# mitrefireline/simfire

Measured on AMD Instinct MI355X. Metric: cell-updates/sec (grid x envs x steps), higher is better.
Workload: dtype u8 status + u8 sprite masks + f64 burn_amounts

## Files before the change

profiles/run_timeline.py:

```python
import ctypes
import sys

import numpy as np

sys.path.insert(0, ".")
from simfire_amd import workloads
from simfire_amd.engine import FireEngine

NAMES = {15: "step start", 1: "interest+ranks", 2: "list+barrierA", 3: "cursor+next fetch issued", 11: "rows arrived", 4: "nb masks, strips",
         5: "SWAR, stores issued", 6: "prefix+frontier list", 7: "walk: winner", 8: "walk: burn/table arrived, update", 9: "walk: stores, fence",
         10: "end of batch", 0: "barrier B (end of step)", 12: "fold", 13: "lines: eligible bits + barrier", 14: "lines: plane work issued", 16: "first batch known", 17: "its rows requested", 18: "next batch known",
         20: "win start", 21: "win rows arrived", 22: "win frontier known", 23: "win winners+req", 24: "win table arrived", 25: "win updated", 26: "win at barrier",
         27: "win thru barrier", 28: "win folded", 30: "launch start", 31: "fire found", 32: "window loaded", 33: "updates done", 34: "written back",
         35: "steps done", 36: "handed back", 37: "result block", 41: "slot written", 42: "placed", 43: "loads issued", 44: "LDS filled",
         45: "cells stored", 46: "bitmap stored", 47: "hist updated", 48: "row written", 49: "state committed",
         50: "lines applied", 51: "next classified", 52: "lines start"}


def main():
    steps, warm = int(sys.argv[1]), int(sys.argv[2])
    env = int(sys.argv[3]) if len(sys.argv) > 3 else -1
    envs = int(sys.argv[4]) if len(sys.argv) > 4 else 256
    c5 = len(sys.argv) > 5 and sys.argv[5] in ("c5", "c3mit")
    c3mit = len(sys.argv) > 5 and sys.argv[5] == "c3mit"
    c4 = len(sys.argv) > 5 and sys.argv[5] == "c4"
    w = workloads.c5(1024, envs) if c5 and not c3mit else (workloads.c4(2048, envs) if c4 else workloads.c3(1024, envs))
    pts = None
    if c3mit:
        pts = np.zeros((steps + warm, w.n_envs, 64, 3), dtype=np.int32)
    elif c5:
        H, W = w.shape
        pts = np.ascontiguousarray(workloads.agent_walk(w.n_envs, w.agents_per_env, H, W, steps + warm).reshape(
            steps + warm, w.n_envs, w.agents_per_env, 4)[..., 1:])

    def run(eng, a, b):
        if c5:
            eng.step_mitigated(pts[a:b])
        else:
            eng.step(b - a)
    eng = FireEngine(M_f=w.M_f, device=0, **w.engine_kwargs())
    eng.set_layers(*w.layers())
    L = eng._L
    L.sf_debug_timeline.argtypes = [ctypes.c_int32, ctypes.c_int32, ctypes.c_void_p]
    L.sf_debug_wave_log.argtypes = [ctypes.c_int32, ctypes.c_void_p]
    log = np.zeros((16384, 4), dtype=np.uint64)
    if env < 0:
        eng.reset(w.init_xy)
        run(eng, 0, warm)
        L.sf_debug_wave_log(1, None)
        run(eng, warm, warm + steps)
        eng.status()
        L.sf_debug_wave_log(0, log.ctypes.data_as(ctypes.c_void_p))
        env = int(np.argmax(log[:envs, 0]))
        print("slowest env", env, "clocks", int(log[env, 0]), "vectors", int(log[env, 1]))
    eng.reset(w.init_xy)
    run(eng, 0, warm)
    L.sf_debug_timeline(env, -1 if len(sys.argv) > 6 and sys.argv[6] == "launch" else steps - 1, None)
    run(eng, warm, warm + steps)
    eng.status()
    tl = np.zeros((16, 64), dtype=np.uint64)
    L.sf_debug_timeline(0, 0, tl.ctypes.data_as(ctypes.c_void_p))
    t0 = min(int(v & np.uint64(0x00FFFFFFFFFFFFFF)) for v in tl[:, 0] if v)
    for wv in range(16):
        ev = [(int(v >> np.uint64(56)), int(v & np.uint64(0x00FFFFFFFFFFFFFF)) - t0) for v in tl[wv] if v]
        print("wave %2d: " % wv + "  ".join("%s@%d" % (NAMES.get(k, str(k)).split(":")[0].split(",")[0][:14], t) for k, t in ev))


if __name__ == "__main__":
    main()
```

simfire_amd/csrc/sf_common.h:

```cpp
#pragma once
#include <hip/hip_runtime.h>

#include <cstdint>

#include "../../include/simfire_hip.h"
#include "../../include/simfire_hip_lab.h"

namespace {


#ifndef SF_WAVES_PER_SIMD
#define SF_WAVES_PER_SIMD 1
#endif
#ifndef SF_WAVES_PER_GROUP
#define SF_WAVES_PER_GROUP 4
#endif
constexpr int kWaves = SF_WAVES_PER_GROUP;
constexpr int kListCap = 384;
constexpr int kSeamPad = 8;
constexpr int kCounterShards = 256;
constexpr int kCounterRow = 16;
constexpr uint32_t FLAG_LIVE = 1u;
constexpr uint32_t FLAG_CAND = 0x100u;

// ... 22 lines not shown
    int Hs;
    long long seam_env;
    int prune_after_quit;
    int VW;
    long long vb_env;
    long long cells_env;
};

__host__ __device__ inline int bl_vec(const Geo &g, int y, int v)
{
    return ((y >> 2) * g.PV + v) * 128 + ((y >> 1) & 1) * 64;
}
__host__ __device__ inline int bl_cell(const Geo &g, int y, int x)
{
    return bl_vec(g, y, x >> 4) + (y & 1) * 16 + (x & 15);
}
constexpr int kBlStatus = 32;

constexpr uint32_t kLoopStop = 0x80000000u;
constexpr uint32_t kJoinClosed = 0x80000000u;
constexpr int kJoinLog = 4096;
constexpr int kTeamMax = 4;
constexpr uint32_t kTeamUnused = 0xFFFFFFFFu;
__host__ __device__ inline int team_xrow(const Geo &g) { return (64 + g.PV * 16 + 127) / 128 * 128; }

struct StepArgs {
    Geo g;
    uint8_t *status;
    uint8_t *age;
    uint8_t *cells;
    double *burn;
    const double *rt;
    unsigned long long *win_hint;
    const double *rtc;
    EnvState *commit;
    EnvState *tmp;
    uint32_t *flags;
    unsigned long long *counters;
    uint8_t *tflags;
    int ring;
    uint32_t *tile_list;
    uint32_t *n_active;
    uint32_t *settled;
    uint8_t *seam;
    uint8_t *tdirty;
    uint8_t *parents;
// ... 186 lines not shown
```

simfire_amd/csrc/sf_run_kernels.h:

```cpp
#pragma once

#include "sf_common.h"
#include "sf_step_kernels.h"

namespace {

constexpr int kMarkDw = 32;
constexpr int kStripDw = 19;
#ifdef SF_NO_PERM_ELIG
#define ELIG(x) elig01(x)
#else
#define ELIG(x) elig01_perm(x)
#endif
constexpr int kRunCtl = 24;
constexpr int kRunMaxD = 4;

typedef uint32_t __attribute__((aligned(1))) u32_unaligned;
typedef uint32_t u32x4 __attribute__((ext_vector_type(4)));

__host__ __device__ inline size_t win_lds_bytes(int n_waves)
{
    const int WR = n_waves * 4;
    return (size_t)WR * 64 * 8 + 8 * 8 * 4 + 128 * 4 + 64 * 4 + (size_t)(WR + 2) * 18 * 4 + (size_t)WR * 16 + (size_t)2 * WR * 64 * 2 + (size_t)2 * WR * 64 +
           (size_t)WR * 64 + (size_t)WR * 8 + 256 * 4;
}
__host__ __device__ inline size_t run_strip_dwords(int n_waves)
{
    const size_t strips = (size_t)n_waves * (64 * kStripDw + kMarkDw), win = (win_lds_bytes(n_waves) + 15) / 16 * 4;
    return strips > win ? strips : win;
}

__host__ __device__ inline size_t run_lds_bytes(const Geo &g, int n_waves, int vcap, int team = 0, int team_rcap = 0)
{
    const int maps = (team || g.VW == 1) ? 4 : 1;
    const int rows = team && team_rcap ? team_rcap + 2 : g.H;
    size_t b = (size_t)maps * rows * g.VW * 8 + (size_t)vcap * 4 + run_strip_dwords(n_waves) * 4 + kRunCtl * 4;
    if (team) b += (size_t)2 * g.PV * 16 + 64 * 4;
// ... 483 lines not shown
        if (TEAM && (tn > 1 || a.team_rcap) && general) fits = cut_bands(tn > 1 && a.team_recut > 0 && a.team_recut < n_steps ? a.team_recut : n_steps - s_begin);
        if (TEAM && a.todo_out && tm == 0 && tid == 0) a.todo_out[e] = fits ? 0 : n_steps - s_begin;
        if (TEAM && !fits) {
            if (!a.todo_out && tid == 0) *reinterpret_cast<volatile uint32_t *>(a.xerr) = 1u;
            if (s_begin > 0 && tm == 0 && tid == 0) a.commit[e] = st;
            return;
        }
    }
    bool has_up = TEAM && tm > 0, has_dn = TEAM && tm + 1 < tn;
    if (TEAM == 2 && tm == 0 && j_s0 < 0 && tid == 0)
        __hip_atomic_store(a.xj + 2 * g.E + 2 + e, (uint32_t)__builtin_amdgcn_s_getreg((20 << 0) | (0 << 6) | (31 << 11)) & 15u, __ATOMIC_RELAXED, __HIP_MEMORY_SCOPE_AGENT);
    auto team_release = [&]() {
        if (TEAM == 2 && a.join_local == 1) asm volatile("s_waitcnt vmcnt(0)" ::: "memory");
        else __builtin_amdgcn_fence(__ATOMIC_RELEASE, "agent");
    };
    auto team_acquire = [&]() { __builtin_amdgcn_fence(__ATOMIC_ACQUIRE, "agent"); };
    bool one_l2 = false;
    bool gave_up = false;
    auto line_up = [&](const uint32_t tag, const bool report) {
        typedef unsigned long long u64;
        int lane = threadIdx.x & 63;
        asm volatile("" : "+v"(lane));
        const uint32_t xcc = (uint32_t)__builtin_amdgcn_s_getreg((20 << 0) | (0 << 6) | (31 << 11)) & 15u;
        if (lane == 0) __hip_atomic_store(a.xg + ((size_t)e * kTeamMax + tm) * 3 + 2, ((u64)tag << 32) | (u64)xcc, __ATOMIC_RELAXED, __HIP_MEMORY_SCOPE_AGENT);
        u64 x = ((u64)tag << 32) | xcc;
        const unsigned long long t0 = __builtin_amdgcn_s_memrealtime();
        for (;;) {
            if (lane < tn) x = __hip_atomic_load(a.xg + ((size_t)e * kTeamMax + lane) * 3 + 2, __ATOMIC_RELAXED, __HIP_MEMORY_SCOPE_AGENT);
            if (__all((uint32_t)(x >> 32) >= tag)) break;
            __builtin_amdgcn_s_sleep(2);
            if (gave_up || __builtin_amdgcn_s_memrealtime() - t0 > a.team_timeout) {
                if (report) {
                    if (lane == 0) *reinterpret_cast<volatile uint32_t *>(a.xerr) = 1u;
                    gave_up = true;
                }
                break;
            }
        }
        one_l2 = __all((uint32_t)(x >> 32) >= tag && ((uint32_t)x & 15u) == xcc) && !a.team_far;
    };
    unsigned long long *vb = vb0, *vf = nullptr, *vl = nullptr, *ve = nullptr;
    auto load_band = [&]() {
        int tid = threadIdx.x;
        asm volatile("" : "+v"(tid));
        const int yoff = TEAM && a.team_rcap ? R0 - 1 : 0;
        vb = vb0 - (long long)yoff * VW;
        vf = fine ? vb + (size_t)lds_rows * VW : nullptr; vl = fine ? vb + (size_t)2 * lds_rows * VW : nullptr;
        ve = fine ? vb + (size_t)3 * lds_rows * VW : nullptr;
        const int y_lo = TEAM && a.team_rcap ? (R0 > 0 ? R0 - 1 : 0) : 0, y_hi = TEAM && a.team_rcap ? (R1 < g.H ? R1 + 1 : g.H) : g.H;
        for (int i = y_lo * VW + tid; i < y_hi * VW; i += nthr) {
            vb[i] = vb_glob[i];
// ... 105 lines not shown
    uint32_t lseq = 0;
    if (loop) {
        if (tid == 0) ctl[18] = __hip_atomic_load(a.loop_done + e, __ATOMIC_RELAXED, __HIP_MEMORY_SCOPE_AGENT);
        __syncthreads();
        lseq = (uint32_t)__builtin_amdgcn_readfirstlane((int)ctl[18]);
        n_steps = 0x7FFFFFFF;
        counts_env(g, e, a.status, a.cells, a.tdirty, a.thist, st.running, st.steps, st.elapsed, a.res_block, a.res_elapsed, nullptr,
                   reinterpret_cast<int32_t (*)[6]>(vlist + vcap));
        if (tid == 0)
            for (int q = 0; q < 6; ++q) ev.tot[q] = a.res_block[e * 8 + 2 + q];
        if (e == 0 && a.mit_k > 0 && lseq > 0) {
            const int n16 = g.E * a.mit_k;
            const u32x4 *src = reinterpret_cast<const u32x4 *>(a.loop_pts_host) + (size_t)(lseq & 1u) * n16;
            u32x4 *cpy = reinterpret_cast<u32x4 *>(a.loop_pts) + (size_t)(lseq & 1u) * n16;
            for (int i = tid; i < n16; i += nthr) {
                u32x4 v;
                asm volatile("global_load_dwordx4 %0, %1, off sc0 sc1\n\ts_waitcnt vmcnt(0)" : "=&v"(v) : "v"(src + i) : "memory");
                if (v.w == lseq) asm volatile("global_store_dwordx4 %0, %1, off sc0 sc1" :: "v"(cpy + i), "v"(v) : "memory");
            }
        }
        __syncthreads();
    }
    unsigned long long join_clk = __builtin_readcyclecounter();
    unsigned long long x_clocks = 0;
    uint32_t x_steps = 0;
    for (int s = s_begin; s < n_steps && (st.running || mit); ++s) {
        const int k = s % 3, kn = (s + 1) % 3;
#ifdef SF_PHASES
        pc.tl = (e == g_timeline_env && s == g_timeline_step) ? g_timeline + wave * 64 : nullptr;
#endif
        auto loop_finish = [&]() {
            __syncthreads();
            if (tid == 0) {
                const int32_t *tot = ev.tot;
                int32_t *row = a.res_block + e * 8;
                row[0] = st.running == 1; row[1] = st.steps;
                for (int q = 0; q < 6; ++q) row[2 + q] = tot[q];
                a.res_elapsed[e] = st.elapsed;
            }
            ++lseq;
            if (wave == 0) {
                uint32_t *stage = strips;
                if (lane == 0) {
                    const int32_t *row = a.res_block + e * 8;
                    const unsigned long long el = (unsigned long long)__double_as_longlong(st.elapsed);
                    stage[0] = (uint32_t)row[0]; stage[1] = (uint32_t)row[1]; stage[2] = (uint32_t)row[2];
                    stage[4] = (uint32_t)row[3]; stage[5] = (uint32_t)row[4]; stage[6] = (uint32_t)row[5];
                    stage[8] = (uint32_t)row[6]; stage[9] = (uint32_t)row[7]; stage[10] = (uint32_t)el;
                    stage[12] = (uint32_t)(el >> 32); stage[13] = 0u; stage[14] = 0u;
                    stage[3] = stage[7] = stage[11] = stage[15] = lseq;
                    __hip_atomic_store(a.loop_done + e, lseq, __ATOMIC_RELAXED, __HIP_MEMORY_SCOPE_AGENT);
                }
// ... 536 lines not shown
                ctl[20] = c > t_cap ? t_cap : (c < (uint32_t)tn ? (uint32_t)tn : c);
                const unsigned long long now = __builtin_readcyclecounter();
                long long per = (long long)((now - join_clk) / (unsigned long long)a.team_recut);
                join_clk = now;
                if (tn > 1) per = (per - a.join_ovh) * tn;
                if (per < a.join_floor) per = a.join_floor;
                const long long left = n_steps - (s + 1);
                const uint32_t b = (uint32_t)((per >> 4) > 0x3FFFF ? 0x3FFFF : (per >> 4)) << 14 | (uint32_t)(left > 0x3FFF ? 0x3FFF : left);
                __hip_atomic_store(a.xj + g.E + e, b, __ATOMIC_RELAXED, __HIP_MEMORY_SCOPE_AGENT);
            }
            if (!recut_now) __syncthreads();
        }
        if (recut_now) {
            store_band();
            team_release();
            __syncthreads();
        }
        if (TEAM == 2 && cut_step && tm == 0) tn_new = __builtin_amdgcn_readfirstlane((int)ctl[20]);
        if (TEAM && tn > 1) {
            if (wave == 0) {
                typedef unsigned long long u64;
                int lane = threadIdx.x & 63;
                asm volatile("" : "+v"(lane));
                const unsigned long long xt0 = a.counters ? __builtin_readcyclecounter() : 0ull;
                const uint32_t epoch = (uint32_t)s + 1u, par = (uint32_t)s & 1u;
                uint8_t *xb_me = a.xbuf + ((size_t)(e * kTeamMax + tm) * 4) * (size_t)a.xrow;
                for (int side = 0; side < 2 && !one_l2; ++side) {
                    if (!(side ? has_dn : has_up)) continue;
                    const int yb = side ? R1 - 1 : R0;
                    u64 *dst = reinterpret_cast<u64 *>(xb_me + (size_t)(side * 2 + par) * a.xrow);
                    for (int v = lane; v < g.PV; v += 64)
                        if ((vb[yb * VW + (v >> 6)] >> (v & 63)) & 1ull) {
                            const uint4 val = *reinterpret_cast<const uint4 *>(ev.cells + bl_vec(g, yb, v) + (yb & 1) * 16);
                            if (one_l2) *reinterpret_cast<uint4 *>(dst + 8 + v * 2) = val;
                            else {
                                __hip_atomic_store(dst + 8 + v * 2, (u64)val.x | ((u64)val.y << 32), __ATOMIC_RELAXED, __HIP_MEMORY_SCOPE_AGENT);
                                __hip_atomic_store(dst + 8 + v * 2 + 1, (u64)val.z | ((u64)val.w << 32), __ATOMIC_RELAXED, __HIP_MEMORY_SCOPE_AGENT);
                            }
                        }
                    if (lane < 3 * VW) {
                        const int which = lane / VW, w = lane - which * VW;
                        const u64 word = (which == 0 ? vb : (which == 1 ? vf : vl))[yb * VW + w];
                        if (one_l2) __hip_atomic_store(dst + lane, word, __ATOMIC_RELAXED, __HIP_MEMORY_SCOPE_WORKGROUP);
                        else __hip_atomic_store(dst + lane, word, __ATOMIC_RELAXED, __HIP_MEMORY_SCOPE_AGENT);
                    }
                }
                asm volatile("s_waitcnt vmcnt(0)" ::: "memory");
                if (lane == 0) {
                    const u64 gv = ((u64)epoch << 32) | (u64)(ctl[3 + k] & 0xFFFFu) | (TEAM == 2 ? (u64)tn_new << 16 : 0ull);
                    if (one_l2) __hip_atomic_store(a.xg + ((size_t)e * kTeamMax + tm) * 3 + par, gv, __ATOMIC_RELAXED, __HIP_MEMORY_SCOPE_WORKGROUP);
                    else __hip_atomic_store(a.xg + ((size_t)e * kTeamMax + tm) * 3 + par, gv, __ATOMIC_RELAXED, __HIP_MEMORY_SCOPE_AGENT);
                }
                u64 x = (u64)epoch << 32;
                {
                    const unsigned long long t0 = __builtin_amdgcn_s_memrealtime();
                    for (;;) {
                        if (lane < tn) x = __hip_atomic_load(a.xg + ((size_t)e * kTeamMax + lane) * 3 + par, __ATOMIC_RELAXED, __HIP_MEMORY_SCOPE_AGENT);
                        if (__all((uint32_t)(x >> 32) == epoch)) break;
                        __builtin_amdgcn_s_sleep(1);
                        if (gave_up || __builtin_amdgcn_s_memrealtime() - t0 > a.team_timeout) {
                            if (lane == 0) *reinterpret_cast<volatile uint32_t *>(a.xerr) = 1u;
                            gave_up = true;
                            break;
                        }
                    }
                }
                const bool live_any = __ballot(lane < tn && (x & 0xFFull)) != 0ull, cand_any = __ballot(lane < tn && (x & 0xFF00ull)) != 0ull;
                if (lane == 0) ctl[3 + k] = (live_any ? FLAG_LIVE : 0u) | (cand_any ? FLAG_CAND : 0u);
                if (TEAM == 2 && cut_step && lane == 0) ctl[20] = (uint32_t)(x >> 16) & 0xFFu;
                for (int side = 0; side < 2 && one_l2; ++side) {
                    if (!(side ? has_dn : has_up)) continue;
                    const int yh = side ? R1 : R0 - 1;
                    for (int v0 = 0; v0 < g.PV; v0 += 64) {
                        const int v = v0 + lane;
                        u64 lo = 0, hi = 0;
                        if (v < g.PV) {
                            const u64 *src = reinterpret_cast<const u64 *>(ev.cells + bl_vec(g, yh, v) + (yh & 1) * 16);
                            lo = __hip_atomic_load(src, __ATOMIC_RELAXED, __HIP_MEMORY_SCOPE_AGENT);
                            hi = __hip_atomic_load(src + 1, __ATOMIC_RELAXED, __HIP_MEMORY_SCOPE_AGENT);
                        }
                        if (v < g.PV) halo[side * g.PV + v] = make_uint4((uint32_t)lo, (uint32_t)(lo >> 32), (uint32_t)hi, (uint32_t)(hi >> 32));
                        const u64 bw = __ballot((lo | hi) != 0ull), fw = __ballot((lo & 0xFFull) != 0ull), lw = __ballot((hi >> 56) != 0ull);
                        if (lane == 0) { vb[yh * VW + (v0 >> 6)] = bw; vf[yh * VW + (v0 >> 6)] = fw; vl[yh * VW + (v0 >> 6)] = lw; }
                    }
                }
                for (int side = 0; side < 2 && !one_l2; ++side) {
                    if (!(side ? has_dn : has_up)) continue;
                    const int nj = side ? tm + 1 : tm - 1, yh = side ? R1 : R0 - 1;
                    const u64 *src = reinterpret_cast<const u64 *>(a.xbuf + ((size_t)(e * kTeamMax + nj) * 4 + (size_t)((side ^ 1) * 2 + par)) * a.xrow);
                    u64 word = 0;
                    if (lane < 3 * VW) word = __hip_atomic_load(src + lane, __ATOMIC_RELAXED, __HIP_MEMORY_SCOPE_AGENT);
                    for (int v0 = 0; v0 < g.PV; v0 += 64) {
                        const int v = v0 + lane;
                        u64 lo = 0, hi = 0;
                        if (v < g.PV) {
                            lo = __hip_atomic_load(src + 8 + v * 2, __ATOMIC_RELAXED, __HIP_MEMORY_SCOPE_AGENT);
                            hi = __hip_atomic_load(src + 8 + v * 2 + 1, __ATOMIC_RELAXED, __HIP_MEMORY_SCOPE_AGENT);
                        }
                        const int wl = v0 >> 6;
                        const u64 bw = (u64)(uint32_t)__builtin_amdgcn_readlane((int)(uint32_t)word, wl) |
                                       ((u64)(uint32_t)__builtin_amdgcn_readlane((int)(uint32_t)(word >> 32), wl) << 32);
                        if (v < g.PV) {
                            const bool on = (bw >> lane) & 1ull;
                            halo[side * g.PV + v] = on ? make_uint4((uint32_t)lo, (uint32_t)(lo >> 32), (uint32_t)hi, (uint32_t)(hi >> 32)) : make_uint4(0, 0, 0, 0);
                        }
                    }
                    if (lane < 3 * VW) {
                        const int which = lane / VW, w = lane - which * VW;
                        (which == 0 ? vb : (which == 1 ? vf : vl))[yh * VW + w] = word;
                    }
                }
                if (a.counters && lane == 0) { x_clocks += __builtin_readcyclecounter() - xt0; x_steps++; }
            }
            __builtin_amdgcn_fence(__ATOMIC_RELEASE, "workgroup", "local");
            __builtin_amdgcn_s_barrier();
            __builtin_amdgcn_fence(__ATOMIC_ACQUIRE, "workgroup", "local");
        }
        st = fold_state(st, ctl[3 + k], g);
        st.running = __builtin_amdgcn_readfirstlane(st.running);
        st.steps = __builtin_amdgcn_readfirstlane(st.steps);
        st.complete = __builtin_amdgcn_readfirstlane(st.complete);
        st.time_quit = __builtin_amdgcn_readfirstlane(st.time_quit);
        if (loop) loop_finish();
        if (TEAM == 2 && cut_step && tn > 1) tn_new = __builtin_amdgcn_readfirstlane((int)ctl[20]);
        if (TEAM == 2 && gave_up) tn_new = tn;
        if ((recut_now || tn_new > tn) && (st.running || mit)) {
            if (TEAM == 2 && tn == 1) {
                store_band();
                team_release();
                __syncthreads();
            }
            if (TEAM == 2 && tn_new > tn && tm == 0 && tid == 0) {
                a.commit[e] = st;
                team_release();
                __hip_atomic_store(a.xcut + e, ((unsigned long long)tn_new << 24) | (unsigned long long)(s + 1), __ATOMIC_RELAXED, __HIP_MEMORY_SCOPE_AGENT);
                atomicAdd(a.xj + 2 * g.E + 1, (uint32_t)(tn_new - tn));
                const uint32_t li = atomicAdd(a.jlog, 1u);
                if (li < (uint32_t)kJoinLog) { a.jlog[1 + 3 * li] = (uint32_t)e; a.jlog[2 + 3 * li] = (uint32_t)(s + 1); a.jlog[3 + 3 * li] = (uint32_t)tn_new; }
            }
            team_acquire();
            if (TEAM == 2) { tn = tn_new; has_up = tm > 0; has_dn = tm + 1 < tn; }
// ... 38 lines not shown
            else a.cost[e] = c32;
        }
    }
    if (TEAM) {
        if (general) store_band();
    } else if (general) {
        for (int i = tid; i < n_words; i += nthr) vb_glob[i] = vb[i];
        if (fine)
            for (int i = tid; i < g.H; i += nthr) {
                vb_glob[(long long)g.E * g.vb_env + i] = vf[i];
                vb_glob[2ll * g.E * g.vb_env + i] = vl[i];
            }
    }
    wpc.note(49);
    if (a.counters && lane == 0) {
        int cw = wave;
        asm volatile("" : "+v"(cw));
        unsigned long long *cs = a.counters + (size_t)((blockIdx.x * 16 + cw) & (kCounterShards - 1)) * kCounterRow;
        if (n_active) atomicAdd(&cs[0], (unsigned long long)n_active);
        if (n_ignite) atomicAdd(&cs[1], (unsigned long long)n_ignite);
        if (n_items_acc) atomicAdd(&cs[2], (unsigned long long)n_items_acc);
        if (n_phase2) atomicAdd(&cs[4], (unsigned long long)n_phase2);
        if (n_vec_done) atomicAdd(&cs[5], (unsigned long long)n_vec_done);
        if (TEAM && x_steps) {
            atomicAdd(&cs[6], (unsigned long long)x_steps | ((unsigned long long)(one_l2 ? x_steps : 0u) << 32));
            atomicAdd(&cs[7], x_clocks);
        }
    }
    if (TEAM && tn > 1) {
        __syncthreads();
        if (tid == 0) {
            __builtin_amdgcn_fence(__ATOMIC_RELEASE, "agent");
            asm volatile("s_waitcnt vmcnt(0)" ::: "memory");
            const uint32_t before = atomicAdd(&a.xdone[e], 1u);
            const bool last = before == (uint32_t)tn - 1u;
            if (last) __builtin_amdgcn_fence(__ATOMIC_ACQUIRE, "agent");
            ctl[0] = last ? 1u : 0u;
        }
        __syncthreads();
        if (!ctl[0]) {
            if (TEAM == 2) continue;
            return;
        }
    }
    if (a.res_block && !(win_result && !general) && !(a.row_valid && !general && n_steps == 0 && !mit)) {
        __syncthreads();
        wpc.note(36);
        counts_env(g, e, a.status, a.cells, a.tdirty, a.thist, st.running, st.steps, st.elapsed, a.res_block, a.res_elapsed, a.res_sink,
                   reinterpret_cast<int32_t (*)[6]>(vlist + vcap));
// ... 92 lines not shown
    for (int e = tid; e < E; e += 1024) atomicAdd(&s_hist[bucket(cost[e])], 1u);
    __syncthreads();
    const uint32_t mine = s_hist[tid];
    const uint32_t incl = wave_scan_incl(mine, lane);
    if (lane == 63) s_wave[wave] = incl;
    __syncthreads();
    uint32_t base = 0;
    for (int w = 0; w < wave; ++w) base += s_wave[w];
    __syncthreads();
    s_hist[tid] = base + incl - mine;
    __syncthreads();
    for (int e = tid; e < E; e += 1024) order[atomicAdd(&s_hist[bucket(cost[e])], 1u)] = (uint32_t)e;
}
#endif

#ifndef SF_RUN_UNIT
__global__ __launch_bounds__(1024) void k_team_plan(int E, int G, int t_min, int t_max, uint32_t ovh, uint32_t floor_c, int scatter, uint32_t *cost, uint32_t *tab, uint32_t *tsize,
                                                    unsigned long long *xg, uint32_t *xdone, int keep_cost, uint32_t *xj, unsigned long long *xcut)
{
    __shared__ uint32_t s_T[1024], s_sum, s_cls[8], s_over;
    const int t = threadIdx.x;
    for (int i = t; i < G; i += 1024) tab[i] = kTeamUnused;
    const uint32_t c = t < E ? cost[t] : 0u;
    for (int i = t; i < E * kTeamMax * 3; i += 1024) xg[i] = 0ull;
    if (t < E) { xdone[t] = 0u; xdone[E + t] = 0u; if (!keep_cost) cost[t] = 0u; }
    if (xj) {
        if (t < E) { xj[t] = 1u; xj[E + t] = 0u; xj[2 * E + 2 + t] = 0xFFFFFFFFu; xcut[t] = 0ull; }
        if (t < 2) xj[2 * E + t] = 0u;
    }
    auto member = [&](int T) -> uint32_t { const uint32_t share = c / (uint32_t)T; return T <= 1 ? c : (share > floor_c ? share : floor_c) + ovh; };
    auto need = [&](uint32_t tgt) -> uint32_t {
        if (t >= E) return 0u;
        if (t_min >= t_max) return (uint32_t)t_min;
        int best = t_min;
        for (int T = t_min; T <= t_max; ++T) {
            if (member(T) <= tgt) return (uint32_t)T;
            if (member(T) < member(best)) best = T;
        }
        return (uint32_t)best;
    };
    auto total = [&](uint32_t v) -> uint32_t {
        __syncthreads();
        if (t == 0) s_sum = 0;
        __syncthreads();
        uint32_t w = v;
        for (int off = 32; off > 0; off >>= 1) w += __shfl_xor(w, off);
        if ((t & 63) == 0 && w) atomicAdd(&s_sum, w);
// ... 79 lines not shown
```

simfire_amd/csrc/sf_step_kernels.h:

```cpp
#pragma once

#include "sf_common.h"

namespace {

constexpr int kSelectThreads = 1024;
#ifndef SF_RUN_UNIT
__global__ __launch_bounds__(kSelectThreads) void k_select(StepArgs a)
{
    __shared__ uint32_t s_base, s_wsum[kSelectThreads / 64];
    const Geo &g = a.g;
    const int per_env = g.TY * g.TX;
    const long long gid = (long long)blockIdx.x * blockDim.x + threadIdx.x;
    const bool valid = gid < (long long)g.E * per_env;
    const int e = valid ? (int)(gid / per_env) : 0;
    const int tile = valid ? (int)(gid - (long long)e * per_env) : 0;
    const int tyw = tile / g.TX, tx = tile - tyw * g.TX;

    const long long fplane = (long long)g.TYp * g.TXp;
    const uint8_t *f_rd = a.tflags + ((long long)a.ring * g.E + e) * fplane;
    uint8_t *f_wr = a.tflags + ((long long)(a.ring ^ 1) * g.E + e) * fplane;
    const long long o = (long long)(tyw + 1) * g.TXp + (tx + 1);
    const EnvState *sp = a.from_commit ? a.commit + e : a.tmp + ((a.launch + 1) & 1) * g.E + e;
    const uint32_t *fp = a.flags + ((a.launch + 2) % 3) * g.E + e;
// ... 56 lines not shown
    __device__ __forceinline__ void mark(int k)
    {
        const unsigned long long n = __builtin_readcyclecounter();
        if (acc && (threadIdx.x & 63) == 0) atomicAdd(&acc[k], (uint32_t)(n - t));
        if (tl && (threadIdx.x & 63) == 0 && tl_n < 64) tl[tl_n++] = ((unsigned long long)k << 56) | (n & 0x00FFFFFFFFFFFFFFull);
        t = n;
    }
    __device__ __forceinline__ void note(int k)
    {
        if (tl && (threadIdx.x & 63) == 0 && tl_n < 64) tl[tl_n++] = ((unsigned long long)k << 56) | (__builtin_readcyclecounter() & 0x00FFFFFFFFFFFFFFull);
    }
#else
    __device__ __forceinline__ void start(uint32_t * = nullptr) {}
    __device__ __forceinline__ void mark(int) {}
    __device__ __forceinline__ void note(int) {}
#endif
};

#ifdef SF_PHASES
__device__ unsigned long long g_wave_log[16384 * 4];
__device__ unsigned long long g_phase[16];
__device__ int g_wave_log_launch = -1;
__device__ int g_timeline_env = -1, g_timeline_step = -1;
__device__ unsigned long long g_timeline[16 * 64];
#endif

struct WalkAcc {
    uint32_t n_active, n_ignite, cand;
    uint32_t edges;
};
__device__ __forceinline__ void acc_merge(WalkAcc &t, const WalkAcc &w)
{
    t.n_active += w.n_active; t.n_ignite += w.n_ignite; t.cand |= w.cand; t.edges |= w.edges;
}

__device__ __forceinline__ uint32_t wave_scan_incl(uint32_t v, int )
{
    v += (uint32_t)__builtin_amdgcn_update_dpp(0, (int)v, 0x111, 0xF, 0xF, true);
    v += (uint32_t)__builtin_amdgcn_update_dpp(0, (int)v, 0x112, 0xF, 0xF, true);
    v += (uint32_t)__builtin_amdgcn_update_dpp(0, (int)v, 0x114, 0xF, 0xF, true);
    v += (uint32_t)__builtin_amdgcn_update_dpp(0, (int)v, 0x118, 0xF, 0xF, true);
    v += (uint32_t)__builtin_amdgcn_update_dpp(0, (int)v, 0x142, 0xA, 0xF, false);
    v += (uint32_t)__builtin_amdgcn_update_dpp(0, (int)v, 0x143, 0xC, 0xF, false);
    return v;
}
__device__ __forceinline__ uint32_t wave_last(uint32_t v) { return (uint32_t)__builtin_amdgcn_readlane((int)v, 63); }
__device__ __forceinline__ uint32_t wave_scan_max(uint32_t v)
// ... 757 lines not shown
```

simfire_amd/csrc/simfire_hip.hip:

```cpp
#include <emmintrin.h>
#include <hip/hip_runtime.h>

#include <cmath>
#include <cstdarg>
#include <cstdint>
#include <cstdio>
#include <cstring>
#include <cstdlib>
#include <algorithm>
#include <map>
#include <string>
#include <tuple>
#include <vector>

#include <dlfcn.h>
#include <rccl/rccl.h>

#include "../../include/simfire_hip.h"
#include "rothermel_dev.h"

static thread_local std::string g_err;
static int fail(int code, const char *fmt, ...)
{
    char buf[512];
// ... 1241 lines not shown
    const Geo &g = s->g;
    TeamGeo t = {};
    if (g.ab != 1 || g.VW != 1 || g.TY > 64 || g.H > 16 * 64 || g.E > 1024 || g.E > s->n_cu || g.dense || !g.diag) return t;
    t.waves = 16; t.vcap = 4096; t.rcap = 0; t.t_min = 1;
    const long long all_vec = (long long)g.H * g.PV;
    if (t.vcap > all_vec) t.vcap = (int)((all_vec + 63) / 64 * 64);
    t.lds = run_lds_bytes(g, t.waves, t.vcap, 1, 0);
    if (t.lds > 160 * 1024 || g.TY < 2) return t;
    if (team_occupancy(s, t, true) == 0) return t;
    t.slots = s->n_cu;
    t.ok = true;
    return t;
}
static int team_buffers(sf_sim *s, const TeamGeo &t)
{
    const Geo &g = s->g;
    if (!s->team_tab || s->team_slots < t.slots) {
        if (s->team_tab) { HIPCHK(hipFree(s->team_tab)); s->team_tab = nullptr; }
        { int rc = dev_alloc(s, &s->team_tab, (size_t)t.slots); if (rc) return rc; }
        s->team_slots = t.slots;
        s->team_plan_ones = 0;
    }
    if (!s->xg) {
        int rc = dev_alloc(s, &s->xg, (size_t)g.E * kTeamMax * 3); if (rc) return rc;
        rc = dev_alloc(s, &s->xbuf, (size_t)g.E * kTeamMax * 4 * team_xrow(g)); if (rc) return rc;
        rc = dev_alloc(s, &s->xdone, (size_t)2 * g.E + 1); if (rc) return rc;
        HIPCHK(hipMemsetAsync(s->xdone, 0, sizeof(uint32_t) * ((size_t)2 * g.E + 1), s->stream));
        rc = dev_alloc(s, &s->team_size, (size_t)g.E); if (rc) return rc;
        HIPCHK(hipHostMalloc(reinterpret_cast<void **>(&s->xerr_pinned), sizeof(uint32_t), hipHostMallocMapped));
        HIPCHK(hipHostGetDevicePointer(reinterpret_cast<void **>(&s->xerr_mapped), s->xerr_pinned, 0));
        *s->xerr_pinned = 0;
        HIPCHK(hipMemsetAsync(s->xbuf, 0, (size_t)g.E * kTeamMax * 4 * team_xrow(g), s->stream));
    }
    return SF_OK;
}

static void team_args(const sf_sim *s, StepArgs &a, int rcap, uint32_t *cost)
{
    a.cost = cost;
    a.team_tab = s->team_tab; a.xg = s->xg; a.xbuf = s->xbuf; a.xdone = s->xdone; a.xerr = s->xerr_mapped;
    a.xrow = team_xrow(s->g); a.team_rcap = rcap;
    a.team_far = s->tune.v[SF_TUNE_TEAM_PLACEMENT] == 2;
    a.order = nullptr;
}

static int launch_k_run_join(sf_sim *s, StepArgs &a, int n_steps, const TeamGeo &t, bool eager)
{
// ... 369 lines not shown
    return SF_OK;
}

extern "C" int sf_history_device(sf_sim *s, void **ptr, int32_t *capacity)
{
    if (!s || !ptr || !capacity) return fail(SF_EINVAL, "sf_history_device: null argument");
    *ptr = s->history; *capacity = s->history_cap;
    return SF_OK;
}

#ifdef SF_PHASES
extern "C" int sf_debug_wave_log(int32_t arm, unsigned long long *out)
{
    if (arm) { int v = -2; return hipMemcpyToSymbol(HIP_SYMBOL(g_wave_log_launch), &v, sizeof v) == hipSuccess ? 0 : -1; }
    int v = -1;
    (void)hipMemcpyToSymbol(HIP_SYMBOL(g_wave_log_launch), &v, sizeof v);
    return hipMemcpyFromSymbol(out, HIP_SYMBOL(g_wave_log), sizeof(unsigned long long) * 16384 * 4) == hipSuccess ? 0 : -1;
}
#endif

#ifdef SF_PHASES
extern "C" int sf_debug_timeline(int32_t env, int32_t step, unsigned long long *out )
{
    if (out) return hipMemcpyFromSymbol(out, HIP_SYMBOL(g_timeline), sizeof(unsigned long long) * 16 * 64) == hipSuccess ? 0 : -1;
    unsigned long long z[16 * 64] = {};
    (void)hipMemcpyToSymbol(HIP_SYMBOL(g_timeline), z, sizeof z);
    (void)hipMemcpyToSymbol(HIP_SYMBOL(g_timeline_step), &step, sizeof step);
    return hipMemcpyToSymbol(HIP_SYMBOL(g_timeline_env), &env, sizeof env) == hipSuccess ? 0 : -1;
}
#endif

#ifdef SF_WIN_PROF
extern "C" int sf_debug_win_prof(unsigned long long *out )
{
    return hipMemcpyFromSymbol(out, HIP_SYMBOL(g_win_prof), sizeof(unsigned long long) * 1024 * 16 * 8) == hipSuccess ? 0 : -1;
}
#endif

#ifdef SF_PHASES
extern "C" int sf_debug_phases(unsigned long long *out16)
{
    if (hipMemcpyFromSymbol(out16, HIP_SYMBOL(g_phase), sizeof(unsigned long long) * 16) != hipSuccess) return -1;
    unsigned long long z[16] = {};
    return hipMemcpyToSymbol(HIP_SYMBOL(g_phase), z, sizeof z) == hipSuccess ? 0 : -1;
}
#endif

extern "C" int sf_step(sf_sim *s, int32_t n_steps) { return step_impl(s, n_steps, nullptr); }
// ... 1294 lines not shown
```

simfire_amd/engine.py:

```python
import ctypes as C
import os

import numpy as np

from . import _lib


def _ptr(a):
    return a.ctypes.data_as(C.c_void_p)


class FireEngine:

    def __init__(self, shape, n_envs=1, max_fire_duration=4, pixel_scale=50.0, update_rate=1.0,
                 max_time=None, attenuate_line_ros=True, diagonal_spread=True, M_f=0.03,
                 particle=(8000.0, 0.0555, 0.01, 32.0), device=0, per_env_terrain=False, variant=None):
        self._L = _lib.load(variant)
        self.H, self.W = int(shape[0]), int(shape[1])
        self.n_envs = int(n_envs)
        h, S_T, S_e, p_p = particle
        self.params = _lib.SfParams(
            n_envs=self.n_envs, height=self.H, width=self.W, max_fire_duration=int(max_fire_duration),
            diagonal_spread=int(bool(diagonal_spread)), attenuate_line_ros=int(bool(attenuate_line_ros)),
            has_max_time=int(max_time is not None), device=int(device), pixel_scale=float(pixel_scale),
# ... 590 lines not shown
        return buf.raw

    def comm_init(self, rank, world_size, unique_id):
        if len(unique_id) != 128:
            raise ValueError("unique_id must be the 128 bytes of comm_unique_id()")
        buf = C.create_string_buffer(bytes(unique_id), 128)
        self._chk(self._L.sf_comm_init(self._h, int(rank), int(world_size), C.cast(buf, C.c_void_p)))

    def allgather_status(self, device_ptr):
        self._chk(self._L.sf_allgather_status(self._h, C.c_void_p(int(device_ptr))))

    def comm_destroy(self):
        self._chk(self._L.sf_comm_destroy(self._h))

    def enable_counters(self, on=True):
        self._chk(self._L.sf_enable_counters(self._h, int(bool(on))))

    def counters(self, reset=False):
        out = np.zeros(16, dtype=np.int64)
        self._chk(self._L.sf_get_counters(self._h, _ptr(out), int(bool(reset))))
        return dict(active_cell_updates=int(out[0]), ignitions=int(out[1]), frontier_items=int(out[2]),
                    active_waves=int(out[3]), frontier_walks=int(out[4]), vectors=int(out[5]),
                    team_boundaries=int(out[6] & 0xFFFFFFFF), team_boundaries_one_l2=int(out[6] >> 32), team_boundary_clocks=int(out[7]),
                    window_updates=int(out[8]), window_waves_looking=int(out[9]))

    def update_status_device(self):
        self._chk(self._L.sf_update_status_device(self._h))


def compute_ros(arrays, device=0):
    L = _lib.load()
    arrs = [np.ascontiguousarray(np.asarray(a, dtype=np.float32).reshape(-1)) for a in arrays]
    if len(arrs) != 17:
        raise ValueError("compute_rate_of_spread takes 17 arrays")
    n = arrs[0].shape[0]
    for a in arrs:
        if a.shape[0] != n:
            raise ValueError("all inputs must have the same length")
    out = np.zeros(n, dtype=np.float64)
    _lib.check(L.sf_compute_ros(n, *[_ptr(a) for a in arrs], _ptr(out), int(device)))
    return out
```

Baseline: 24190 billion.

## Let team members wait only on neighbours at step boundaries when fire stays live

Adds a 'near' mode to the team step-boundary exchange. When the team shares one L2, the step is not a recut, and the member's own fire is live with candidates, it polls only its adjacent members' words instead of all members, and assumes live/cand flags are set. Exchange words move to a four-slot ring per member (indexed by step), so a fast member can run ahead without overwriting words a slower member still needs. Up/down halo row loads are interleaved, and counters and timeline instrumentation for the boundary phases are added. The change risks correctness if a non-neighbour's state matters, and SF_TEAM_CHECK is provided to detect that.

```diff
diff --git a/profiles/run_timeline.py b/profiles/run_timeline.py
--- a/profiles/run_timeline.py
+++ b/profiles/run_timeline.py
@@ -14,7 +14,8 @@
          27: "win thru barrier", 28: "win folded", 30: "launch start", 31: "fire found", 32: "window loaded", 33: "updates done", 34: "written back",
          35: "steps done", 36: "handed back", 37: "result block", 41: "slot written", 42: "placed", 43: "loads issued", 44: "LDS filled",
          45: "cells stored", 46: "bitmap stored", 47: "hist updated", 48: "row written", 49: "state committed",
-         50: "lines applied", 51: "next classified", 52: "lines start"}
+         50: "lines applied", 51: "next classified", 52: "lines start",
+         53: "own word out", 54: "neighbours' words in", 55: "all words in", 56: "halo rows in", 57: "folded"}
 
 
 def main():
@@ -55,15 +56,22 @@
         print("slowest env", env, "clocks", int(log[env, 0]), "vectors", int(log[env, 1]))
     eng.reset(w.init_xy)
     run(eng, 0, warm)
-    L.sf_debug_timeline(env, -1 if len(sys.argv) > 6 and sys.argv[6] == "launch" else steps - 1, None)
+    L.sf_debug_timeline(env, -1 if len(sys.argv) > 6 and sys.argv[6] == "launch" else steps - 2, None)
     run(eng, warm, warm + steps)
     eng.status()
-    tl = np.zeros((16, 64), dtype=np.uint64)
+    tl = np.zeros((4, 16, 64), dtype=np.uint64)
     L.sf_debug_timeline(0, 0, tl.ctypes.data_as(ctypes.c_void_p))
-    t0 = min(int(v & np.uint64(0x00FFFFFFFFFFFFFF)) for v in tl[:, 0] if v)
-    for wv in range(16):
-        ev = [(int(v >> np.uint64(56)), int(v & np.uint64(0x00FFFFFFFFFFFFFF)) - t0) for v in tl[wv] if v]
-        print("wave %2d: " % wv + "  ".join("%s@%d" % (NAMES.get(k, str(k)).split(":")[0].split(",")[0][:14], t) for k, t in ev))
+    t0 = min(int(v & np.uint64(0x00FFFFFFFFFFFFFF)) for v in tl[:, :, 0].ravel() if v)
+    for m in range(4):
+        if not tl[m].any():
+            continue
+        print("member %d" % m)
+        for wv in range(16):
+            ev = [(int(v >> np.uint64(56)), int(v & np.uint64(0x00FFFFFFFFFFFFFF)) - t0) for v in tl[m, wv] if v]
+            print("wave %2d: " % wv + "  ".join("%s@%d" % (NAMES.get(k, str(k)).split(":")[0].split(",")[0][:14], t) for k, t in ev))
+        w0 = {k: t for k, t in ((int(v >> np.uint64(56)), int(v & np.uint64(0x00FFFFFFFFFFFFFF)) - t0) for v in tl[m, 0] if v)}
+        if 0 in w0 and 57 in w0:
+            print("  barrier B -> fold: %d clocks" % (w0[57] - w0[0]))
 
 
 if __name__ == "__main__":
diff --git a/profiles/team_boundary_split.py b/profiles/team_boundary_split.py
--- /dev/null
+++ b/profiles/team_boundary_split.py
@@ -0,0 +1,40 @@
+#!/usr/bin/env python3
+import os
+import sys
+
+import numpy as np
+
+sys.path.insert(0, ".")
+import bench
+from simfire_amd import workloads
+
+steps = int(sys.argv[1]) if len(sys.argv) > 1 else 1000
+warm = int(sys.argv[2]) if len(sys.argv) > 2 else 20
+names = sys.argv[3].split(",") if len(sys.argv) > 3 else ["c3", "c4", "c5"]
+lib = os.environ.get("SIMFIRE_HIP_LIB")
+print("library:", os.path.relpath(lib) if lib else "(product)", "| updates", steps, "after", warm, flush=True)
+for name in names:
+    w = bench.make_workload(name, 1024, {"c3": 256, "c4": 128, "c5": 64}[name], 0)
+    pts = None
+    if name == "c5":
+        H, W = w.shape
+        pts = bench.AgentPoints(workloads.agent_walk(w.n_envs, w.agents_per_env, H, W, steps + warm), w.n_envs, w.agents_per_env, 0)
+    eng = bench.make_engine(w, 0)
+    eng.enable_counters(True)
+    for rnd in range(2):
+        eng.reset(w.init_xy)
+        bench.run_steps(eng, warm, 0, pts)
+        eng.status()
+        eng.counters(reset=True)
+        ms = bench.timed_steps(eng, steps, warm, pts)
+    c = eng.counters()
+    sizes = eng.team_sizes()
+    n = max(c["team_boundaries"], 1)
+    print(f"{name}: {ms / steps * 1e3:6.2f} us per update (counters on); team sizes {np.bincount(sizes, minlength=5).tolist()}; "
+          f"boundaries {c['team_boundaries']} ({c['team_boundaries_one_l2']} through one L2, {c['team_boundaries_near']} waited for neighbours only); "
+          f"clocks each {c['team_boundary_clocks'] / n:.0f} = own word out {c['team_boundary_publish_clocks'] / n:.0f} + first look {c['team_boundary_first_poll_clocks'] / n:.0f}"
+          f" + wait {c['team_boundary_wait_clocks'] / n:.0f} + rows to halo {c['team_boundary_rows_clocks'] / n:.0f}; "
+          f"wait's share {c['team_boundary_wait_clocks'] / max(c['team_boundary_clocks'], 1):.2f}; "
+          f"came last (first look found every word) {c['team_boundaries_came_last'] / n:.2f} of the boundaries, "
+          f"of those last at the boundary before too {c['team_boundaries_came_last_again'] / max(c['team_boundaries_came_last'], 1):.2f}", flush=True)
+    eng.close()
diff --git a/simfire_amd/csrc/sf_common.h b/simfire_amd/csrc/sf_common.h
--- a/simfire_amd/csrc/sf_common.h
+++ b/simfire_amd/csrc/sf_common.h
@@ -68,6 +68,7 @@
 constexpr int kJoinLog = 4096;
 constexpr int kTeamMax = 4;
 constexpr uint32_t kTeamUnused = 0xFFFFFFFFu;
+constexpr int kXgRow = kTeamMax + 1;
 __host__ __device__ inline int team_xrow(const Geo &g) { return (64 + g.PV * 16 + 127) / 128 * 128; }
 
 struct StepArgs {
diff --git a/simfire_amd/csrc/sf_run_kernels.h b/simfire_amd/csrc/sf_run_kernels.h
--- a/simfire_amd/csrc/sf_run_kernels.h
+++ b/simfire_amd/csrc/sf_run_kernels.h
@@ -12,7 +12,9 @@
 #else
 #define ELIG(x) elig01_perm(x)
 #endif
-constexpr int kRunCtl = 24;
+constexpr int kRunCtl = 40;
+constexpr int kXsClk = 24;
+constexpr int kXsCnt = 32;
 constexpr int kRunMaxD = 4;
 
 typedef uint32_t __attribute__((aligned(1))) u32_unaligned;
@@ -542,11 +544,11 @@
         int lane = threadIdx.x & 63;
         asm volatile("" : "+v"(lane));
         const uint32_t xcc = (uint32_t)__builtin_amdgcn_s_getreg((20 << 0) | (0 << 6) | (31 << 11)) & 15u;
-        if (lane == 0) __hip_atomic_store(a.xg + ((size_t)e * kTeamMax + tm) * 3 + 2, ((u64)tag << 32) | (u64)xcc, __ATOMIC_RELAXED, __HIP_MEMORY_SCOPE_AGENT);
+        if (lane == 0) __hip_atomic_store(a.xg + ((size_t)e * kTeamMax + tm) * kXgRow + kTeamMax, ((u64)tag << 32) | (u64)xcc, __ATOMIC_RELAXED, __HIP_MEMORY_SCOPE_AGENT);
         u64 x = ((u64)tag << 32) | xcc;
         const unsigned long long t0 = __builtin_amdgcn_s_memrealtime();
         for (;;) {
-            if (lane < tn) x = __hip_atomic_load(a.xg + ((size_t)e * kTeamMax + lane) * 3 + 2, __ATOMIC_RELAXED, __HIP_MEMORY_SCOPE_AGENT);
+            if (lane < tn) x = __hip_atomic_load(a.xg + ((size_t)e * kTeamMax + lane) * kXgRow + kTeamMax, __ATOMIC_RELAXED, __HIP_MEMORY_SCOPE_AGENT);
             if (__all((uint32_t)(x >> 32) >= tag)) break;
             __builtin_amdgcn_s_sleep(2);
             if (gave_up || __builtin_amdgcn_s_memrealtime() - t0 > a.team_timeout) {
@@ -698,12 +700,10 @@
         __syncthreads();
     }
     unsigned long long join_clk = __builtin_readcyclecounter();
-    unsigned long long x_clocks = 0;
-    uint32_t x_steps = 0;
     for (int s = s_begin; s < n_steps && (st.running || mit); ++s) {
         const int k = s % 3, kn = (s + 1) % 3;
 #ifdef SF_PHASES
-        pc.tl = (e == g_timeline_env && s == g_timeline_step) ? g_timeline + wave * 64 : nullptr;
+        pc.tl = (e == g_timeline_env && s == g_timeline_step) ? g_timeline + ((TEAM ? tm : 0) * 16 + wave) * 64 : nullptr;
 #endif
         auto loop_finish = [&]() {
             __syncthreads();
@@ -1286,8 +1286,14 @@
                 typedef unsigned long long u64;
                 int lane = threadIdx.x & 63;
                 asm volatile("" : "+v"(lane));
-                const unsigned long long xt0 = a.counters ? __builtin_readcyclecounter() : 0ull;
-                const uint32_t epoch = (uint32_t)s + 1u, par = (uint32_t)s & 1u;
+                unsigned long long xt = a.counters ? __builtin_readcyclecounter() : 0ull;
+                auto xmark = [&](int q) {
+                    if (!a.counters) return;
+                    const unsigned long long now = __builtin_readcyclecounter();
+                    if (lane == 0) reinterpret_cast<u64 *>(ctl + kXsClk)[q] += now - xt;
+                    xt = now;
+                };
+                const uint32_t epoch = (uint32_t)s + 1u, par = (uint32_t)s & 1u, slot = (uint32_t)s & (uint32_t)(kTeamMax - 1);
                 uint8_t *xb_me = a.xbuf + ((size_t)(e * kTeamMax + tm) * 4) * (size_t)a.xrow;
                 for (int side = 0; side < 2 && !one_l2; ++side) {
                     if (!(side ? has_dn : has_up)) continue;
@@ -1310,17 +1316,31 @@
                     }
                 }
                 asm volatile("s_waitcnt vmcnt(0)" ::: "memory");
+                const uint32_t own = ctl[3 + k] & 0xFFFFu;
                 if (lane == 0) {
-                    const u64 gv = ((u64)epoch << 32) | (u64)(ctl[3 + k] & 0xFFFFu) | (TEAM == 2 ? (u64)tn_new << 16 : 0ull);
-                    if (one_l2) __hip_atomic_store(a.xg + ((size_t)e * kTeamMax + tm) * 3 + par, gv, __ATOMIC_RELAXED, __HIP_MEMORY_SCOPE_WORKGROUP);
-                    else __hip_atomic_store(a.xg + ((size_t)e * kTeamMax + tm) * 3 + par, gv, __ATOMIC_RELAXED, __HIP_MEMORY_SCOPE_AGENT);
-                }
+                    const u64 gv = ((u64)epoch << 32) | (u64)own | (TEAM == 2 ? (u64)tn_new << 16 : 0ull);
+                    if (one_l2) __hip_atomic_store(a.xg + ((size_t)e * kTeamMax + tm) * kXgRow + slot, gv, __ATOMIC_RELAXED, __HIP_MEMORY_SCOPE_WORKGROUP);
+                    else __hip_atomic_store(a.xg + ((size_t)e * kTeamMax + tm) * kXgRow + slot, gv, __ATOMIC_RELAXED, __HIP_MEMORY_SCOPE_AGENT);
+                }
+#ifdef SF_TEAM_WAIT_ALL
+                const bool near = false;
+#else
+                const bool near = one_l2 && !cut_step && s + 1 < n_steps && (own & FLAG_LIVE) && (own & FLAG_CAND);
+#endif
+                pc.note(53);
+                const bool ask = lane < tn && (!near || lane == tm - 1 || lane == tm + 1);
+                xmark(0);
                 u64 x = (u64)epoch << 32;
                 {
                     const unsigned long long t0 = __builtin_amdgcn_s_memrealtime();
-                    for (;;) {
-                        if (lane < tn) x = __hip_atomic_load(a.xg + ((size_t)e * kTeamMax + lane) * 3 + par, __ATOMIC_RELAXED, __HIP_MEMORY_SCOPE_AGENT);
-                        if (__all((uint32_t)(x >> 32) == epoch)) break;
+                    for (bool first = true;; first = false) {
+                        if (ask) x = __hip_atomic_load(a.xg + ((size_t)e * kTeamMax + lane) * kXgRow + slot, __ATOMIC_RELAXED, __HIP_MEMORY_SCOPE_AGENT);
+                        const bool all_in = __all((uint32_t)(x >> 32) == epoch);
+                        if (first && a.counters) {
+                            xmark(1);
+                            if (lane == 0) { ctl[kXsCnt + 1] += all_in ? 1u : 0u; ctl[kXsCnt + 2] += all_in ? ctl[kXsCnt + 3] : 0u; ctl[kXsCnt + 3] = all_in ? 1u : 0u; }
+                        }
+                        if (all_in) break;
                         __builtin_amdgcn_s_sleep(1);
                         if (gave_up || __builtin_amdgcn_s_memrealtime() - t0 > a.team_timeout) {
                             if (lane == 0) *reinterpret_cast<volatile uint32_t *>(a.xerr) = 1u;
@@ -1329,22 +1349,36 @@
                         }
                     }
                 }
-                const bool live_any = __ballot(lane < tn && (x & 0xFFull)) != 0ull, cand_any = __ballot(lane < tn && (x & 0xFF00ull)) != 0ull;
+#ifdef SF_TEAM_CHECK
+                if (near && !gave_up) {
+                    u64 y = 0ull;
+                    if (ask) y = __hip_atomic_load(a.xg + ((size_t)e * kTeamMax + lane) * kXgRow + ((slot + 1u) & (uint32_t)(kTeamMax - 1)), __ATOMIC_RELAXED, __HIP_MEMORY_SCOPE_AGENT);
+                    if (!__all((uint32_t)(y >> 32) <= epoch) && lane == 0) *reinterpret_cast<volatile uint32_t *>(a.xerr) = 1u;
+                }
+#endif
+                xmark(2);
+                pc.note(near ? 54 : 55);
+                const bool live_any = near || __ballot(lane < tn && (x & 0xFFull)) != 0ull, cand_any = near || __ballot(lane < tn && (x & 0xFF00ull)) != 0ull;
                 if (lane == 0) ctl[3 + k] = (live_any ? FLAG_LIVE : 0u) | (cand_any ? FLAG_CAND : 0u);
                 if (TEAM == 2 && cut_step && lane == 0) ctl[20] = (uint32_t)(x >> 16) & 0xFFu;
-                for (int side = 0; side < 2 && one_l2; ++side) {
-                    if (!(side ? has_dn : has_up)) continue;
-                    const int yh = side ? R1 : R0 - 1;
-                    for (int v0 = 0; v0 < g.PV; v0 += 64) {
-                        const int v = v0 + lane;
-                        u64 lo = 0, hi = 0;
-                        if (v < g.PV) {
+                for (int v0 = 0; v0 < g.PV && one_l2; v0 += 64) {
+                    const int v = v0 + lane;
+                    u64 lo[2] = {0ull, 0ull}, hi[2] = {0ull, 0ull};
+#pragma unroll
+                    for (int side = 0; side < 2; ++side) {
+                        const int yh = side ? R1 : R0 - 1;
+                        if ((side ? has_dn : has_up) && v < g.PV) {
                             const u64 *src = reinterpret_cast<const u64 *>(ev.cells + bl_vec(g, yh, v) + (yh & 1) * 16);
-                            lo = __hip_atomic_load(src, __ATOMIC_RELAXED, __HIP_MEMORY_SCOPE_AGENT);
-                            hi = __hip_atomic_load(src + 1, __ATOMIC_RELAXED, __HIP_MEMORY_SCOPE_AGENT);
+                            lo[side] = __hip_atomic_load(src, __ATOMIC_RELAXED, __HIP_MEMORY_SCOPE_AGENT);
+                            hi[side] = __hip_atomic_load(src + 1, __ATOMIC_RELAXED, __HIP_MEMORY_SCOPE_AGENT);
                         }
-                        if (v < g.PV) halo[side * g.PV + v] = make_uint4((uint32_t)lo, (uint32_t)(lo >> 32), (uint32_t)hi, (uint32_t)(hi >> 32));
-                        const u64 bw = __ballot((lo | hi) != 0ull), fw = __ballot((lo & 0xFFull) != 0ull), lw = __ballot((hi >> 56) != 0ull);
+                    }
+#pragma unroll
+                    for (int side = 0; side < 2; ++side) {
+                        if (!(side ? has_dn : has_up)) continue;
+                        const int yh = side ? R1 : R0 - 1;
+                        if (v < g.PV) halo[side * g.PV + v] = make_uint4((uint32_t)lo[side], (uint32_t)(lo[side] >> 32), (uint32_t)hi[side], (uint32_t)(hi[side] >> 32));
+                        const u64 bw = __ballot((lo[side] | hi[side]) != 0ull), fw = __ballot((lo[side] & 0xFFull) != 0ull), lw = __ballot((hi[side] >> 56) != 0ull);
                         if (lane == 0) { vb[yh * VW + (v0 >> 6)] = bw; vf[yh * VW + (v0 >> 6)] = fw; vl[yh * VW + (v0 >> 6)] = lw; }
                     }
                 }
@@ -1374,13 +1408,16 @@
                         (which == 0 ? vb : (which == 1 ? vf : vl))[yh * VW + w] = word;
                     }
                 }
-                if (a.counters && lane == 0) { x_clocks += __builtin_readcyclecounter() - xt0; x_steps++; }
+                pc.note(56);
+                xmark(3);
+                if (a.counters && lane == 0) { ctl[kXsCnt] += near ? 1u : 0u; ctl[kXsCnt + 4] += 1u; }
             }
             __builtin_amdgcn_fence(__ATOMIC_RELEASE, "workgroup", "local");
             __builtin_amdgcn_s_barrier();
             __builtin_amdgcn_fence(__ATOMIC_ACQUIRE, "workgroup", "local");
         }
         st = fold_state(st, ctl[3 + k], g);
+        pc.note(57);
         st.running = __builtin_amdgcn_readfirstlane(st.running);
         st.steps = __builtin_amdgcn_readfirstlane(st.steps);
         st.complete = __builtin_amdgcn_readfirstlane(st.complete);
@@ -1465,9 +1502,18 @@
         if (n_items_acc) atomicAdd(&cs[2], (unsigned long long)n_items_acc);
         if (n_phase2) atomicAdd(&cs[4], (unsigned long long)n_phase2);
         if (n_vec_done) atomicAdd(&cs[5], (unsigned long long)n_vec_done);
-        if (TEAM && x_steps) {
+        if (TEAM && cw == 0 && ctl[kXsCnt + 4]) {
+            const unsigned long long *xs = reinterpret_cast<const unsigned long long *>(ctl + kXsClk);
+            const uint32_t x_steps = ctl[kXsCnt + 4];
             atomicAdd(&cs[6], (unsigned long long)x_steps | ((unsigned long long)(one_l2 ? x_steps : 0u) << 32));
-            atomicAdd(&cs[7], x_clocks);
+            atomicAdd(&cs[7], xs[0] + xs[1] + xs[2] + xs[3]);
+            atomicAdd(&cs[10], (unsigned long long)ctl[kXsCnt]);
+            atomicAdd(&cs[11], xs[2]);
+            atomicAdd(&cs[12], xs[0]);
+            atomicAdd(&cs[13], xs[1]);
+            atomicAdd(&cs[14], xs[3]);
+            atomicAdd(&cs[15], (unsigned long long)ctl[kXsCnt + 1] | ((unsigned long long)ctl[kXsCnt + 2] << 32));
+            for (int q = kXsClk; q < kXsCnt + 5; ++q) ctl[q] = 0u;
         }
     }
     if (TEAM && tn > 1) {
@@ -1606,7 +1652,7 @@
     const int t = threadIdx.x;
     for (int i = t; i < G; i += 1024) tab[i] = kTeamUnused;
     const uint32_t c = t < E ? cost[t] : 0u;
-    for (int i = t; i < E * kTeamMax * 3; i += 1024) xg[i] = 0ull;
+    for (int i = t; i < E * kTeamMax * kXgRow; i += 1024) xg[i] = 0ull;
     if (t < E) { xdone[t] = 0u; xdone[E + t] = 0u; if (!keep_cost) cost[t] = 0u; }
     if (xj) {
         if (t < E) { xj[t] = 1u; xj[E + t] = 0u; xj[2 * E + 2 + t] = 0xFFFFFFFFu; xcut[t] = 0ull; }
diff --git a/simfire_amd/csrc/sf_step_kernels.h b/simfire_amd/csrc/sf_step_kernels.h
--- a/simfire_amd/csrc/sf_step_kernels.h
+++ b/simfire_amd/csrc/sf_step_kernels.h
@@ -102,7 +102,7 @@
 __device__ unsigned long long g_phase[16];
 __device__ int g_wave_log_launch = -1;
 __device__ int g_timeline_env = -1, g_timeline_step = -1;
-__device__ unsigned long long g_timeline[16 * 64];
+__device__ unsigned long long g_timeline[4 * 16 * 64];
 #endif
 
 struct WalkAcc {
diff --git a/simfire_amd/csrc/simfire_hip.hip b/simfire_amd/csrc/simfire_hip.hip
--- a/simfire_amd/csrc/simfire_hip.hip
+++ b/simfire_amd/csrc/simfire_hip.hip
@@ -1287,7 +1287,7 @@
         s->team_plan_ones = 0;
     }
     if (!s->xg) {
-        int rc = dev_alloc(s, &s->xg, (size_t)g.E * kTeamMax * 3); if (rc) return rc;
+        int rc = dev_alloc(s, &s->xg, (size_t)g.E * kTeamMax * kXgRow); if (rc) return rc;
         rc = dev_alloc(s, &s->xbuf, (size_t)g.E * kTeamMax * 4 * team_xrow(g)); if (rc) return rc;
         rc = dev_alloc(s, &s->xdone, (size_t)2 * g.E + 1); if (rc) return rc;
         HIPCHK(hipMemsetAsync(s->xdone, 0, sizeof(uint32_t) * ((size_t)2 * g.E + 1), s->stream));
@@ -1703,8 +1703,9 @@
 #ifdef SF_PHASES
 extern "C" int sf_debug_timeline(int32_t env, int32_t step, unsigned long long *out )
 {
-    if (out) return hipMemcpyFromSymbol(out, HIP_SYMBOL(g_timeline), sizeof(unsigned long long) * 16 * 64) == hipSuccess ? 0 : -1;
-    unsigned long long z[16 * 64] = {};
+    static_assert(kTeamMax == 4, "g_timeline holds four members' lines");
+    if (out) return hipMemcpyFromSymbol(out, HIP_SYMBOL(g_timeline), sizeof(unsigned long long) * kTeamMax * 16 * 64) == hipSuccess ? 0 : -1;
+    static unsigned long long z[kTeamMax * 16 * 64] = {};
     (void)hipMemcpyToSymbol(HIP_SYMBOL(g_timeline), z, sizeof z);
     (void)hipMemcpyToSymbol(HIP_SYMBOL(g_timeline_step), &step, sizeof step);
     return hipMemcpyToSymbol(HIP_SYMBOL(g_timeline_env), &env, sizeof env) == hipSuccess ? 0 : -1;
diff --git a/simfire_amd/engine.py b/simfire_amd/engine.py
--- a/simfire_amd/engine.py
+++ b/simfire_amd/engine.py
@@ -636,7 +636,10 @@
         return dict(active_cell_updates=int(out[0]), ignitions=int(out[1]), frontier_items=int(out[2]),
                     active_waves=int(out[3]), frontier_walks=int(out[4]), vectors=int(out[5]),
                     team_boundaries=int(out[6] & 0xFFFFFFFF), team_boundaries_one_l2=int(out[6] >> 32), team_boundary_clocks=int(out[7]),
-                    window_updates=int(out[8]), window_waves_looking=int(out[9]))
+                    window_updates=int(out[8]), window_waves_looking=int(out[9]),
+                    team_boundaries_near=int(out[10]), team_boundary_wait_clocks=int(out[11]), team_boundary_publish_clocks=int(out[12]),
+                    team_boundary_first_poll_clocks=int(out[13]), team_boundary_rows_clocks=int(out[14]),
+                    team_boundaries_came_last=int(out[15] & 0xFFFFFFFF), team_boundaries_came_last_again=int(out[15] >> 32))
 
     def update_status_device(self):
         self._chk(self._L.sf_update_status_device(self._h))
```

Result: slower. 23710 billion (-2.0%).
